# Anony-CFFM/CFFM

Measured on AMD Instinct MI355X. Metric: training examples/sec, frappe 10-field dim32; embedding-gather %HBM roofline, higher is better.
Workload: dtype f32; 1 GPU; frappe shape: synthetic libfm, 10 fields, 5382 features, inner/outer dim 32, batch 256 per GPU, selu, Adagrad lr 0.05, square_loss (README.md:28); global_batch=256, id_distribution=uniform, tables=replicated, parallelism=single

## Files before the change

cffm_amd/csrc/conv.hip:

```cpp
#include <cstdlib>
#include <cstring>

#include "internal.hpp"

#include <type_traits>

#include <stdlib.h>
#include "inner_body.hpp"
#include "head_body.hpp"
#include "sort_body.hpp"

#define KSTEP 32
#define WG_KM 64

__device__ __forceinline__ int64_t xcd_tile(int64_t per_xcd) {
    const int64_t id = blockIdx.x;
    return (id & 7) * per_xcd + (id >> 3);
}
__host__ __device__ static inline int64_t xcd_per(int64_t tiles) { return (tiles + 7) / 8; }

struct RowPos { int b, y, x; };
__device__ __forceinline__ RowPos row_pos(int64_t m, int lgSo) {
    RowPos p;
    const int So = 1 << lgSo;
// ... 1684 lines not shown
                PHASE_MARK(1 + l);
                fused_layer_fwd<NT, G, ACT, LGSO>(fa.conv[l], b, smem, CL(l - 1), CL(l));
            });
        } else {
            for (int l = 1; l < live; ++l) {
                if (lds_act) lds_barrier(); else __syncthreads();
                PHASE_MARK(1 + l);
                fused_layer_fwd<NT, G, ACT>(fa.conv[l], b, smem, CL(l - 1), CL(l));
            }
        }
        if (lds_act) lds_barrier(); else __syncthreads();
        PHASE_MARK(1 + live);
        head_fwd_body<NW, ACT, false, F_, D_>(fa.head, b, smem, lds_act, c0_off, c1_off);
        PHASE_MARK(2 + live);
    };
    if constexpr (CS) {
        static_assert(!CS || 4096 / (CS ? F_ : 1) <= 2 * 256, "two passes over a grid of 256 workgroups cover every accepted B");
        if ((int)blockIdx.x < fa.B) example((int)blockIdx.x);
        if (const int b = blockIdx.x + gridDim.x; b < fa.B) {
            __syncthreads();
            example(b);
        }
    } else {
        for (int b = blockIdx.x; b < fa.B; b += gridDim.x) {
            if (b != (int)blockIdx.x) __syncthreads();
            example(b);
        }
    }
#ifdef CFFM_PHASE_TIMERS
    if (threadIdx.x == 0) cffm_wg_times[2 * blockIdx.x + 1] = wall_clock64();
#endif
}

template <int NT, int F_, int D_, int NW>
__device__ __forceinline__ void conv0_fact_bwd_body(const DgradArgs& a, float* __restrict__ slabW, float* __restrict__ slabB,
                                                    int64_t slab_stride, char* smem, int wg, int nwg) {
    constexpr int PP = NT * 16, S = 16, NTH = 64 * NW, XQ = 16 / NW;
    const int F = F_ ? F_ : a.F, D = D_ ? D_ : a.D, Dp = D + 1, P = F_ ? F_ * (F_ - 1) / 2 : a.P, F2 = 2 * F;
    const int TP = S * PP + 16;
    float* Wl = reinterpret_cast<float*>(smem);
    float* T = Wl + 4 * PP * PP;
    float* part = T + 2 * F * TP;
    float* dEi = part + NW * 16 * 32;
    float* dEj = dEi + 32 * 16;
    float* bred = dEj + 32 * 16;
    float* rs = bred + NW * PP;
    float* Es = rs + 2 * F;
    const int tid = threadIdx.x, lane = tid & 63, wave = tid >> 6, r = lane & 15, kk = lane >> 4;
    float* sw = slabW + (int64_t)wg * slab_stride;
    float* sb = slabB + (int64_t)wg * slab_stride;
    PHASE_MARKB(12, wg);
    {
        const float4* wsrc = reinterpret_cast<const float4*>(a.W);
        for (int i = tid; i < 4 * PP * PP / 4; i += NTH) reinterpret_cast<float4*>(Wl)[i] = wsrc[i];
        for (int e = tid; e < 4 * (PP - P) * PP; e += NTH) {
            const int tap = e / ((PP - P) * PP), o = e - tap * ((PP - P) * PP);
            sw[(tap * PP + P) * PP + o] = 0.f;
        }
    }
    bool first = true;
    float bacc[NT];
#pragma unroll
    for (int nt = 0; nt < NT; ++nt) bacc[nt] = 0.f;

    for (int b = wg; b < a.B; b += nwg) {
        __syncthreads();
        {
// ... 184 lines not shown
                }
            }
#pragma unroll
            for (int ct = 0; ct < 2; ++ct)
#pragma unroll
                for (int j = 0; j < 4; ++j) part[(wave * 16 + kk * 4 + j) * 32 + ct * 16 + r] = acc[ct][j];
        }
        PHASE_MARKB(18, wg);
        if (tid < 2 * F) {
            const int f = tid % F;
            float sacc = 0.f;
            if (tid < F) { for (int h = 0; h < D; ++h) sacc += Es[f * Dp + h]; }
            else { for (int h = 0; h < D; ++h) sacc += Es[f * Dp + h] * a.dt1[(int64_t)b * a.t1w + h]; }
            rs[tid] = sacc;
        }
        __syncthreads();
        for (int e = tid; e < 16 * 32; e += NTH) {
            float v = part[e];
#pragma unroll
            for (int w = 1; w < NW; ++w) v += part[512 * w + e];
            dEj[(e & 31) * 16 + (e >> 5)] = v;
        }
        __syncthreads();
        PHASE_MARKB(19, wg);
        for (int e = tid; e < F * D; e += NTH) {
            const int f = e / D, h = e - f * D, lo = h & 1, hh = h >> 1;
            float R = 0.f, Q = 0.f;
            for (int j = f + 1; j < F; ++j) R += rs[j];
            for (int i = 0; i < f; ++i) Q += rs[F + i];
            a.dprev[(int64_t)b * F * D + e] = (dEi[(lo * F + f) * 16 + hh] + dEj[(lo * F + f) * 16 + hh])
                                              + a.dt1[(int64_t)b * a.t1w + h] * R + Q;
        }
        first = false;
    }
    PHASE_MARKB(20, wg);
    __syncthreads();
#pragma unroll
    for (int nt = 0; nt < NT; ++nt) {
        float v = bacc[nt];
        v += __shfl_xor(v, 16, 64);
        v += __shfl_xor(v, 32, 64);
        if (kk == 0) bred[wave * PP + nt * 16 + r] = v;
    }
    __syncthreads();
    if (tid < PP) {
        float v = bred[tid];
#pragma unroll
        for (int w = 1; w < NW; ++w) v += bred[w * PP + tid];
        sb[tid] = v;
    }
    if (first) {
        for (int e = tid; e < 4 * PP * PP; e += NTH) sw[e] = 0.f;
    }
    PHASE_MARKB(25, wg);
}

template <int NT, int F_, int D_, int NW>
__global__ __launch_bounds__(64 * NW) void conv0_fact_bwd_kernel(DgradArgs a, float* __restrict__ slabW,
                                                              float* __restrict__ slabB, int64_t slab_stride) {
    extern __shared__ __attribute__((aligned(16))) char smem[];
    conv0_fact_bwd_body<NT, F_, D_, NW>(a, slabW, slabB, slab_stride, smem, blockIdx.x, gridDim.x);
}

template <int NT, int RM, bool L0, int HALVES, int ACTC = -1>
__device__ __forceinline__ void dgrad_taps_body(const DgradArgs& a, int wg, char* smem, int64_t m_lo = 0, int64_t m_end = -1,
                                                int tiles = 1, int tid_in = -1) {
// ... 468 lines not shown
struct Conv01Args {
    DgradArgs d0;
    float *slabW0, *slabB0;
    int64_t stride0;
    DgradArgs d1;
    WgradArgs w1, w2, w3;
    int n2, n3;
};

template <int NT, int F_, int D_, int ACT>
__global__ __launch_bounds__(1024) void conv01_bwd_kernel(Conv01Args a) {
    extern __shared__ __attribute__((aligned(16))) char smem[];
    const int b = blockIdx.x, grp = __builtin_amdgcn_readfirstlane((int)(threadIdx.x >> 8)), ltid = threadIdx.x & 255;
    PHASE_MARKB(40, b);
    dgrad_taps_body<NT, 1, false, 4, ACT>(a.d1, b, smem, 0, -1, 4);
    PHASE_MARKB(41, b);
    {
        char* gsm = smem + (size_t)grp * (64 * NT * 16 * 4);
        const WgradArgs& w = grp == 0 ? a.w1 : (grp == 1 ? a.w2 : a.w3);
        const int nsl = grp == 0 ? (int)gridDim.x : (grp == 1 ? a.n2 : a.n3);
        const int slab = grp == 1 ? b - ((int)gridDim.x - a.n2) : b;
        const bool mine = grp < 3 && slab >= 0 && slab < nsl;
        int64_t m_lo = 0, m_hi = 0;
        if (mine) {
            const int64_t per = grp == 0 ? (1ll << (2 * w.lgSo)) : CFFM_TOP_SLAB_ROWS;
            m_lo = (int64_t)slab * per;
            m_hi = min(w.Mtot, m_lo + per);
            if (m_hi < m_lo) m_hi = m_lo;
        }
        wgrad_taps_body<NT, false, 1, ACT>(w, mine ? slab : 0, nsl, gsm, m_lo, m_hi, ltid, mine);
    }
    __syncthreads();
    PHASE_MARKB(42, b);
    conv0_fact_bwd_body<NT, F_, D_, 16>(a.d0, a.slabW0, a.slabB0, a.stride0, smem, b, (int)gridDim.x);
}

struct BwdTopArgs {
    HeadBwdArgs hb;
    DgradArgs d[2];
    WgradArgs w[2];
    int lgSo[2];
    int n_layers;
    int wgrad_here;
    InnerBwdArgs ib;
    int n_inner;
    int n_keys;
    const int32_t* rank_ids;
    unsigned long long* keys_sorted;
    int n_rows;
};

template <int NT, int ACT = -1>
__global__ __launch_bounds__(256) void bwd_top_kernel(BwdTopArgs a) {
    extern __shared__ __attribute__((aligned(16))) char smem[];
    __shared__ float dh1s[CFFM_HEAD_UNITS];
    __shared__ float dt1s[1024];
    __shared__ float red[4];
    const int bid = blockIdx.x;
#ifdef CFFM_PHASE_TIMERS
    if (threadIdx.x == 0) cffm_wg_times[2 * blockIdx.x] = wall_clock64();
#endif
    if (bid < a.n_inner) {
        PHASE_MARKB(36, bid);
        const float L = head_bwd_loss(a.hb, false, red);
        __syncthreads();
        PHASE_MARKB(37, bid);
        if (a.rank_ids != nullptr && a.n_keys == 0) {
            for (int b = bid; b < a.hb.B; b += a.n_inner) rank_keys_body<4>(a.rank_ids, a.n_rows, b, a.hb.g.F, a.hb.g.M, a.keys_sorted, smem);
        }
        PHASE_MARKB(38, bid);
        inner_bwd_body<ACT>(a.ib, bid, a.n_inner, smem, L);
        PHASE_MARKB(39, bid);
#ifdef CFFM_PHASE_TIMERS
        if (threadIdx.x == 0) cffm_wg_times[2 * blockIdx.x + 1] = wall_clock64();
#endif
        return;
    }
    if (bid < a.n_inner + a.n_keys) {
        for (int b = bid - a.n_inner; b < a.hb.B; b += a.n_keys) rank_keys_body<4>(a.rank_ids, a.n_rows, b, a.hb.g.F, a.hb.g.M, a.keys_sorted, smem);
#ifdef CFFM_PHASE_TIMERS
        if (threadIdx.x == 0) cffm_wg_times[2 * blockIdx.x + 1] = wall_clock64();
#endif
        return;
    }
    const int b = bid - a.n_inner - a.n_keys;
    PHASE_MARKB(0, b);
    HeadBwdState st;
    head_bwd_begin(a.hb, b, st);
    PHASE_MARKB(1, b);
    const float L = head_bwd_loss(a.hb, b == 0, red);
    PHASE_MARKB(2, b);
    if (b < a.hb.B)
        head_bwd_example<ACT>(a.hb, b, st, b, head_dout(a.hb.loss, a.hb.out[b], a.hb.y[b], 1.f / (float)a.hb.Bg, L), dh1s, dt1s);
    PHASE_MARKB(3, b);
    head_bwd_end(a.hb, b, st);
    PHASE_MARKB(4, b);
    for (int t = 0; t < a.n_layers; ++t) {
        __syncthreads();
        const int64_t rows = 1ll << (2 * a.lgSo[t]);
        const int64_t m_lo = (int64_t)b * rows, m_hi = b < a.hb.B ? m_lo + rows : m_lo;
        if (a.wgrad_here) wgrad_taps_body<NT, false, 1, ACT>(a.w[t], b, (int)gridDim.x - a.n_inner - a.n_keys, smem, m_lo, m_hi);
        PHASE_MARKB(5 + 2 * t, b);
        for (int64_t m0 = m_lo; m0 < m_hi; m0 += 16) dgrad_taps_body<NT, 1, false, 1, ACT>(a.d[t], 0, smem, m0, m_hi);
        PHASE_MARKB(6 + 2 * t, b);
// ... 1261 lines not shown
        default: return CFFM_ERR_UNSUPPORTED;
    }
}

template <int NT>
static int launch_bwd_top(const BwdTopArgs& a, size_t lds, hipStream_t st) {
    return with_readme_act<NT>(a.hb.g.act, [&](auto act) {
        constexpr int ACT = decltype(act)::value;
        int rc = set_lds(bwd_top_kernel<NT, ACT>, lds);
        if (rc) return rc;
        hipLaunchKernelGGL((bwd_top_kernel<NT, ACT>), dim3(a.n_inner + a.n_keys + 256), dim3(256), lds, st, a);
        CFFM_CHECK_LAUNCH();
        return 0;
    });
}

int cffm_bwd_top_impl(const StepCtx& c, const float* y, int64_t B_global, const BwdOpts& o, hipStream_t st, int* next_layer) {
    const cffm_shape_t* s = c.s;
    const Geo& g = c.g;
    const int32_t B = c.B;
    BwdTopArgs a;
    memset(&a, 0, sizeof(a));
    a.hb = c.head_bwd_args(y, B_global, o);
    const int first = bwd_top_first_layer(s);
    a.wgrad_here = (top_wgrad_deferred(s, B) || bwd_fused01_ok(s, B)) ? 0 : 1;
    a.n_layers = 0;
    for (int l = g.live - 1; l >= first; --l) {
        a.d[a.n_layers] = c.dgrad_args(l);
        a.w[a.n_layers] = c.wgrad_args(l);
        a.lgSo[a.n_layers] = a.d[a.n_layers].lgSo;
        ++a.n_layers;
    }
    a.ib = c.inner_bwd_args(&a.n_inner);
    a.ib.dout = nullptr;
    a.ib.y = y; a.ib.invB = 1.f / (float)B_global;
    if (o.rank_ids != nullptr && s->F <= RANK_MAXF && (int64_t)B * s->F <= 4096) {
        a.rank_ids = o.rank_ids; a.n_rows = B * s->F;
        a.keys_sorted = c.at<unsigned long long>(c.wl.sort_vals);
        a.n_keys = 256;
    }
    size_t lds = (size_t)(WGT_SUB * g.Pp) * 4 + 16;
    if (inner_bwd_lds(g) > lds) lds = inner_bwd_lds(g);
    *next_layer = first - 1;
    return with_int<NT4>(g.Pp / 16, [&](auto nt) { return launch_bwd_top<CV(nt)>(a, lds, st); });
}

int cffm_conv_bwd_impl(const StepCtx& c, int l, hipStream_t st, const ConvBwdOpts& o) {
    const Geo& g = c.g;
    if (l < 0 || l >= g.live) return CFFM_ERR_BAD_SHAPE;
    if (int rc = cffm_conv_lds_check(c)) return rc;
    const SlabRange& sr = c.conv_slab(l);
    const int nsl = sr.nslab;
    WgradArgs wa = c.wgrad_args(l);
    DgradArgs da = c.dgrad_args(l);
    const ConvBwdChoice k = conv_bwd_choice(g, c.B, l, nsl, conv_b3_on());
    const KC &kw = k.wgrad, &kd = k.dgrad;
    if (kw.family == CFFM_CHOICE_UNSUPPORTED || kd.family == CFFM_CHOICE_UNSUPPORTED) return CFFM_ERR_UNSUPPORTED;
    if (o.with_top_wgrad && !k.paired) return CFFM_ERR_UNSUPPORTED;
    const bool tiled_w = kw.family == CFFM_WGRAD_TILE_ALL || kw.family == CFFM_WGRAD_TILE_GROUP;
    if (o.rs && !(tiled_w && kd.family == CFFM_DGRAD_TILE_PACKED)) return CFFM_ERR_UNSUPPORTED;
    if (k.paired) {
        InnerBwdArgs ib{};
        int n_i = 0;
        const bool inner = o.carry_inner != nullptr && c.s->inner_conv;
        if (inner) ib = c.inner_bwd_args(&n_i);
        TopWgrad tw;
// ... 69 lines not shown
extern "C" int cffm_outer_conv0_bwd(const cffm_shape_t* s, const float* theta, void* ws, int32_t B, void* stream) {
    int rc = check_shape(s);
    if (rc) return rc;
    if (B <= 0 || !s->outer_conv) return 0;
    return cffm_conv_bwd_impl(StepCtx(s, B, theta, ws), 0, (hipStream_t)stream);
}
extern "C" int cffm_conv_bwd(const cffm_shape_t* s, const float* theta, void* ws, int32_t B, int32_t layer, void* stream) {
    int rc = check_shape(s);
    if (rc) return rc;
    if (B <= 0 || !s->outer_conv) return 0;
    if (layer < 1) return CFFM_ERR_BAD_SHAPE;
    return cffm_conv_bwd_impl(StepCtx(s, B, theta, ws), layer, (hipStream_t)stream);
}
bool cffm_wide_regather_ok(const cffm_shape_t* s) {
    if (check_shape(s) || !s->inner_conv || !s->outer_conv) return false;
    const Geo g = make_geo(s);
    return conv0_tile_fwd_ok(g) && conv0_tile_wgrad_ok(g) && conv0_tile_dgrad2_ok(g) && g.K == g.D && (g.K == 32 || g.K == 64) &&
           cffm_giw_lds_ok();
}

int cffm_conv01_bwd_impl(const StepCtx& c, hipStream_t st) {
    const cffm_shape_t* s = c.s;
    const Geo& g = c.g;
    const int32_t B = c.B;
    if (!bwd_fused01_ok(s, B) || g.live != 4 || !conv0_fact_bwd_ok(g)) return CFFM_ERR_UNSUPPORTED;
    Conv01Args a;
    memset(&a, 0, sizeof(a));
    const WgradArgs w0 = c.wgrad_args(0);
    a.d0 = c.dgrad_args(0);
    a.slabW0 = w0.slabW; a.slabB0 = w0.slabB; a.stride0 = w0.slab_stride;
    a.d1 = c.dgrad_args(1);
    a.w1 = c.wgrad_args(1); a.w2 = c.wgrad_args(2); a.w3 = c.wgrad_args(3);
    a.n2 = c.conv_slab(2).nslab; a.n3 = c.conv_slab(3).nslab;
    if (c.conv_slab(0).nslab != 256 || c.conv_slab(1).nslab != 256 || a.n2 > 256 || a.n3 > 256 ||
        (int64_t)a.n2 * CFFM_TOP_SLAB_ROWS < a.w2.Mtot || (int64_t)a.n3 * CFFM_TOP_SLAB_ROWS < a.w3.Mtot)
        return CFFM_ERR_UNSUPPORTED;
    {
        const void* must[] = {a.d0.dC, a.d0.W, a.d0.Cprev, a.d0.dt1, a.d0.dprev, a.slabW0, a.slabB0, a.d1.dC, a.d1.W, a.d1.Cprev,
                              a.d1.dt1, a.d1.dprev, a.w1.in, a.w1.dC, a.w1.slabW, a.w1.slabB, a.w2.in, a.w2.dC, a.w2.slabW,
                              a.w2.slabB, a.w3.in, a.w3.dC, a.w3.slabW, a.w3.slabB};
        for (const void* q : must)
            if (q == nullptr) return CFFM_ERR_BAD_SHAPE;
        if (a.d0.Mtot <= 0 || a.d1.Mtot <= 0 || a.w1.Mtot <= 0 || a.w2.Mtot <= 0 || a.w3.Mtot <= 0 || a.n2 < 1 || a.n3 < 1 ||
            a.stride0 <= 0 || a.w1.slab_stride <= 0 || a.w2.slab_stride <= 0 || a.w3.slab_stride <= 0)
            return CFFM_ERR_BAD_SHAPE;
    }
    const int NW = 16, PP = g.Pp;
    const size_t lds = conv0_fact_bwd_lds(PP, g.F, g.D);
#define CFFM_C01_LAUNCH(NTV, FV, DV, ACTV)                                                                       \
    do {                                                                                                         \
        int rc = set_lds(conv01_bwd_kernel<NTV, FV, DV, ACTV>, lds);                                             \
        if (rc) return rc;                                                                                       \
        hipLaunchKernelGGL((conv01_bwd_kernel<NTV, FV, DV, ACTV>), dim3(256), dim3(1024), lds, st, a);          \
    } while (0)
    const int nt = PP / 16;
    if (frappe_shape(g)) CFFM_C01_LAUNCH(3, 10, 32, CFFM_ACT_SELU);
    else if (nt == 3) CFFM_C01_LAUNCH(3, 0, 0, -1);
    else if (nt == 2) CFFM_C01_LAUNCH(2, 0, 0, -1);
    else CFFM_C01_LAUNCH(1, 0, 0, -1);
#undef CFFM_C01_LAUNCH
    CFFM_CHECK_LAUNCH();
    return 0;
}

bool cffm_fwd_all_ok(const cffm_shape_t* s, int32_t B) {
    const Geo g = make_geo(s);
// ... 54 lines not shown
```

cffm_amd/csrc/inner_body.hpp:

```cpp
#pragma once
#include "common.hpp"

struct InnerUnit {
    float x0, x1, I0, I1, z0, z1, s0, s1, eix, eiy, ejx, ejy;
    int i, j;
};

__device__ __forceinline__ InnerUnit inner_unit(const float* E, const uint32_t* lut, int p, int t, int K,
                                                const float* cw, const float* cb, int act) {
    InnerUnit u;
    const uint32_t ij = lut[p];
    u.i = ij & 0xffff; u.j = ij >> 16;
    const float2 ei = *reinterpret_cast<const float2*>(&E[u.i * K + 2 * t]);
    const float2 ej = *reinterpret_cast<const float2*>(&E[u.j * K + 2 * t]);
    u.eix = ei.x; u.eiy = ei.y; u.ejx = ej.x; u.ejy = ej.y;
    u.I0 = ei.x * ej.x; u.I1 = ei.y * ej.y;
    u.x0 = act_f(u.I0, act); u.x1 = act_f(u.I1, act);
    u.z0 = u.x0 * cw[0] + u.x1 * cw[2] + cb[0];
    u.z1 = u.x0 * cw[1] + u.x1 * cw[3] + cb[1];
    const float mp = fmaxf(u.x0, u.x1);
    u.s0 = act_pos(fmaxf(u.z0, 0.f), act) + mp;
    u.s1 = act_pos(fmaxf(u.z1, 0.f), act) + mp;
    return u;
}
// ... 77 lines not shown
    float cw[4] = {cw_g[0], cw_g[1], cw_g[2], cw_g[3]};
    float cb[2] = {cb_g[0], cb_g[1]};
    const int K2 = g.K / 2, units = g.P * K2;
    const float2* wd2 = reinterpret_cast<const float2*>(wd);
    const float2 w2_first = (int)threadIdx.x < units ? wd2[threadIdx.x] : make_float2(0.f, 0.f);
    __syncthreads();
    const float invK2 = 1.f / (float)K2;
    float part = 0.f;
    for (int u = threadIdx.x; u < units; u += blockDim.x) {
        const int p = fast_div(u, invK2), t = u - p * K2;
        const InnerUnit v = inner_unit(E, lut, p, t, g.K, cw, cb, act);
        const float2 w2 = u == (int)threadIdx.x ? w2_first : wd2[u];
        part += v.s0 * w2.x + v.s1 * w2.y;
    }
    const float tot = block_sum(part, red);
    if (threadIdx.x == 0) inner_out[b] = tot + bd[0];
}

struct InnerBwdArgs {
    Geo g;
    int B;
    const float *Ei, *dout, *cw, *cb, *wd;
    const float *out, *y;
    int loss;
    float invB;
    float* dEi;
    float *slab_cw, *slab_cb, *slab_dw, *slab_db;
    int64_t slab_stride;
    const int32_t* idx = nullptr;
    int idxM = 0;
    int idxStride = 0;
};

template <int ACTC = -1>
__device__ __forceinline__ void inner_bwd_body(const InnerBwdArgs& a, int slab, int nslab, char* smem, float L = 1.f) {
    const Geo& g = a.g;
    const int act = ACTC >= 0 ? ACTC : g.act;
    const int B = a.B;
    const float* __restrict__ Ei = a.Ei; const float* __restrict__ dout = a.dout;
    const float* __restrict__ cw_g = a.cw; const float* __restrict__ cb_g = a.cb; const float* __restrict__ wd = a.wd;
    float* __restrict__ dEi = a.dEi;
    float* __restrict__ slab_cw = a.slab_cw + slab * a.slab_stride; float* __restrict__ slab_cb = a.slab_cb + slab * a.slab_stride;
    float* __restrict__ slab_dw = a.slab_dw + slab * a.slab_stride; float* __restrict__ slab_db = a.slab_db + slab * a.slab_stride;
    const int FK = g.F * g.K;
    float* E = reinterpret_cast<float*>(smem);
    float* dE = E + FK;
    uint32_t* lut = reinterpret_cast<uint32_t*>(dE + 4 * FK);
    float* red = reinterpret_cast<float*>(lut + g.Pp);
    const int wave = threadIdx.x >> 6;
    build_pair_lut(lut, g.F, g.Pp);
    if (threadIdx.x < 8) slab_cw[threadIdx.x] = 0.f;
    if (threadIdx.x < 4) slab_db[threadIdx.x] = 0.f;
    float cw[4] = {cw_g[0], cw_g[1], cw_g[2], cw_g[3]};
    float cb[2] = {cb_g[0], cb_g[1]};
    const int K2 = g.K / 2, units = g.P * K2;
    const float invK2 = 1.f / (float)K2;
    float gcw[4] = {0.f, 0.f, 0.f, 0.f}, gcb[2] = {0.f, 0.f}, gdb = 0.f;
    constexpr int UPRE = 4;
    const float2* wd2 = reinterpret_cast<const float2*>(wd);
    float2 w2p[UPRE];
#pragma unroll
    for (int k = 0; k < UPRE; ++k) {
        const int u = threadIdx.x + k * blockDim.x;
        w2p[k] = u < units ? wd2[u] : make_float2(0.f, 0.f);
    }
    bool first = true;
    for (int b = slab; b < B; b += nslab) {
// ... 17 lines not shown
        auto unit_step = [&](int u, float2 w2) {
            const int p = fast_div(u, invK2), t = u - p * K2;
            const InnerUnit v = inner_unit(E, lut, p, t, g.K, cw, cb, act);
            const int64_t wi = (int64_t)p * g.K + 2 * t;
            float2 acc2 = first ? make_float2(0.f, 0.f) : *reinterpret_cast<float2*>(&slab_dw[wi]);
            acc2.x += v.s0 * db; acc2.y += v.s1 * db;
            *reinterpret_cast<float2*>(&slab_dw[wi]) = acc2;
            const float ds0 = db * w2.x, ds1 = db * w2.y;
            const float dz0 = ds0 * act_relu_grad(fmaxf(v.z0, 0.f), act);
            const float dz1 = ds1 * act_relu_grad(fmaxf(v.z1, 0.f), act);
            gcw[0] += dz0 * v.x0; gcw[1] += dz1 * v.x0; gcw[2] += dz0 * v.x1; gcw[3] += dz1 * v.x1;
            gcb[0] += dz0; gcb[1] += dz1;
            const float dmp = ds0 + ds1;
            const bool firstmax = v.x0 >= v.x1;
            const float dx0 = dz0 * cw[0] + dz1 * cw[1] + (firstmax ? dmp : 0.f);
            const float dx1 = dz0 * cw[2] + dz1 * cw[3] + (firstmax ? 0.f : dmp);
            const float dI0 = dx0 * act_grad_f(v.I0, act), dI1 = dx1 * act_grad_f(v.I1, act);
            atomicAdd(&myE[v.i * g.K + 2 * t], dI0 * v.ejx);
            atomicAdd(&myE[v.i * g.K + 2 * t + 1], dI1 * v.ejy);
            atomicAdd(&myE[v.j * g.K + 2 * t], dI0 * v.eix);
            atomicAdd(&myE[v.j * g.K + 2 * t + 1], dI1 * v.eiy);
        };
#pragma unroll
        for (int k = 0; k < UPRE; ++k) {
            const int u = threadIdx.x + k * blockDim.x;
            if (u < units) unit_step(u, w2p[k]);
        }
        for (int u = threadIdx.x + UPRE * blockDim.x; u < units; u += blockDim.x) unit_step(u, wd2[u]);
        if (threadIdx.x == 0) gdb += db;
        __syncthreads();
        for (int i = threadIdx.x; i < FK; i += blockDim.x)
            dEi[(int64_t)b * FK + i] = ((dE[i] + dE[FK + i]) + dE[2 * FK + i]) + dE[3 * FK + i];
        first = false;
    }
    if (first) {
        for (int64_t i = threadIdx.x; i < (int64_t)g.P * g.K; i += blockDim.x) slab_dw[i] = 0.f;
    }
    float r[7] = {gcw[0], gcw[1], gcw[2], gcw[3], gcb[0], gcb[1], gdb};
#pragma unroll
    for (int q = 0; q < 7; ++q) r[q] = wave_sum(r[q]);
    __syncthreads();
    if ((threadIdx.x & 63) == 0) {
#pragma unroll
        for (int q = 0; q < 7; ++q) dE[wave * 8 + q] = r[q];
    }
    __syncthreads();
    if (threadIdx.x == 0) {
        const int nw = blockDim.x >> 6;
#pragma unroll
        for (int q = 0; q < 7; ++q) {
            float t = 0.f;
            for (int w = 0; w < nw; ++w) t += dE[w * 8 + q];
            r[q] = t;
        }
        for (int q = 0; q < 4; ++q) slab_cw[q] = r[q];
        slab_cb[0] = r[4]; slab_cb[1] = r[5];
        slab_db[0] = r[6];
    }
}
```

cffm_amd/csrc/optim.hip:

```cpp
#include "internal.hpp"

#include <cmath>
#include <cstring>
#include <rocprim/device/device_radix_sort.hpp>

#define REDUCE_GROUPS 64
static inline int reduce_slab_wgs(int64_t n) { return (int)((n / 4 + REDUCE_GROUPS - 1) / REDUCE_GROUPS); }
__device__ __forceinline__ void reduce_slabs_body(int bid, const float* __restrict__ gpart, int64_t n, const SlabPlan& sp,
                                                  float* __restrict__ grad, float* __restrict__ theta,
                                                  float* __restrict__ acc, float lr) {
    __shared__ float4 part[4][REDUCE_GROUPS];
    const int g = threadIdx.x & 63, q = threadIdx.x >> 6;
    const int64_t i = ((int64_t)bid * REDUCE_GROUPS + g) * 4;
    float4 s = make_float4(0.f, 0.f, 0.f, 0.f);
    if (i < n) {
        int hit = 0;
        for (int r = 1; r < sp.n; ++r)
            if (i >= sp.r[r].off) hit = r;
        const SlabRange rg = sp.r[hit];
        const float4* src = reinterpret_cast<const float4*>(gpart + rg.base + (i - rg.off));
        const int64_t stride = rg.len / 4;
        const int per = (rg.nslab + 3) / 4, k0 = q * per, k1 = min(rg.nslab, k0 + per);
#pragma unroll 8
        for (int k = k0; k < k1; ++k) {
            const float4 v = src[(int64_t)k * stride];
            s.x += v.x; s.y += v.y; s.z += v.z; s.w += v.w;
        }
    }
    part[q][g] = s;
    __syncthreads();
    if (q != 0 || i >= n) return;
#pragma unroll
    for (int e = 1; e < 4; ++e) {
        const float4 p = part[e][g];
        s.x += p.x; s.y += p.y; s.z += p.z; s.w += p.w;
    }
    *reinterpret_cast<float4*>(grad + i) = s;
    if (theta != nullptr) {
        float4 a = *reinterpret_cast<float4*>(acc + i), t = *reinterpret_cast<float4*>(theta + i);
        a.x += s.x * s.x; a.y += s.y * s.y; a.z += s.z * s.z; a.w += s.w * s.w;
        t.x -= lr * s.x / sqrtf(a.x); t.y -= lr * s.y / sqrtf(a.y); t.z -= lr * s.z / sqrtf(a.z); t.w -= lr * s.w / sqrtf(a.w);
        *reinterpret_cast<float4*>(acc + i) = a;
        *reinterpret_cast<float4*>(theta + i) = t;
    }
}

__global__ __launch_bounds__(256) void reduce_slabs_kernel(const float* __restrict__ gpart, int64_t n, SlabPlan sp,
                                                           float* __restrict__ grad, float* __restrict__ theta,
                                                           float* __restrict__ acc, float lr) {
    reduce_slabs_body(blockIdx.x, gpart, n, sp, grad, theta, acc, lr);
}

__device__ __forceinline__ float late_scale(const LateScale& ls) {
    return ls.on ? 1.f / sqrtf(ls.sum[0] * ls.inv_Bg + 1e-10f) : 1.f;
}

struct AdagradRule {
    float lr;
    __device__ __forceinline__ bool slot() const { return true; }
// ... 203 lines not shown
    return 0;
}

__global__ __launch_bounds__(256) void pack_keys_kernel(const int32_t* __restrict__ ids, unsigned long long* keys, int64_t n,
                                                        int64_t id_stride, int M) {
    const int64_t i = (int64_t)blockIdx.x * 256 + threadIdx.x;
    if (i < n) {
        const int raw = ids[i * id_stride];
        keys[i] = ((unsigned long long)(unsigned)((raw < 0 || raw >= M) ? M : raw) << 32) | (unsigned long long)i;
    }
}

#include "sort_body.hpp"

__global__ __launch_bounds__(256) void small_sort_kernel(const unsigned long long* __restrict__ in,
                                                         unsigned long long* __restrict__ out, int n, int id_bits) {
    extern __shared__ __attribute__((aligned(16))) char smem[];
    small_sort_body(in, nullptr, out, n, id_bits, smem);
}

struct SparseArgs {
    const unsigned long long* keys;
    int64_t n;
    int M, K, D;
    const float *dEi, *dEo, *dfb;
    int64_t sEi, sEo, sfb;
    int run_len;
    int64_t run_stride;
    float inv_run_len;
};
enum { T_INNER = 0, T_OUTER = 1, T_BIAS = 2 };
static const cffm_tables_t NO_TABLES = {nullptr, nullptr, nullptr};

template <class Sink>
__device__ __forceinline__ void segment_walk(int bid, const SparseArgs& a, const Sink& sink) {
    const unsigned long long* __restrict__ keys = a.keys;
    const int64_t n = a.n;
    const int M = a.M, K = a.K, D = a.D;
    const float* __restrict__ dEi = a.dEi; const float* __restrict__ dEo = a.dEo; const float* __restrict__ dfb = a.dfb;
    const int64_t pos = (int64_t)bid * 4 + (threadIdx.x >> 6);
    const int lane = threadIdx.x & 63;
    if (pos >= n) return;
    const int id = (int)(keys[pos] >> 32);
    if (pos > 0 && (int)(keys[pos - 1] >> 32) == id) return;
    if (id < 0 || id >= M) return;
    const int W = (dEi ? K : 0) + (dEo ? D : 0) + 1;
    const int Ki = dEi ? K : 0;
    for (int c0 = 0; c0 < W; c0 += 64) {
        const int c = c0 + lane;
        float g = 0.f;
        if (c < W) {
            for (int64_t q = pos; q < n; ++q) {
                const unsigned long long kq = keys[q];
                if ((int)(kq >> 32) != id) break;
                int64_t sl = (int64_t)(kq & 0xffffffffull);
                int64_t boff = 0;
                if (a.run_len > 0) {
                    const int blk = fast_div((int)sl, a.inv_run_len);
                    boff = (int64_t)blk * a.run_stride;
                    sl -= (int64_t)blk * a.run_len;
                }
                g += c < Ki ? dEi[boff + sl * a.sEi + c] : (c < W - 1 ? dEo[boff + sl * a.sEo + (c - Ki)] : dfb[boff + sl * a.sfb]);
            }
            typename Sink::At at;
            if (c < Ki) at = sink.at(id, T_INNER, c);
            else if (c < W - 1) at = sink.at(id, T_OUTER, c - Ki);
            else at = sink.at(id, T_BIAS, 0);
            sink(at, g);
        }
    }
}

__device__ __forceinline__ int64_t row_off(int K, int D, int id, int t, int col) {
    if (t == T_INNER) return (int64_t)id * K + col;
    if (t == T_OUTER) return (int64_t)id * D + col;
    return id;
}
__device__ __forceinline__ float* table_of(const cffm_tables_t& T, int t) {
    if (t == T_INNER) return T.inner_emb;
    if (t == T_OUTER) return T.outer_emb;
    return T.feat_bias;
}
template <class Rule, bool LATE>
struct ApplySink {
    cffm_tables_t w, s;
    int K, D;
    Rule rule;
    float gscale = 1.f;
    struct At { float *w, *s; };
    __device__ __forceinline__ At at(int id, int t, int col) const {
        const int64_t o = row_off(K, D, id, t, col);
        return {table_of(w, t) + o, rule.slot() ? table_of(s, t) + o : nullptr};
    }
    __device__ __forceinline__ void operator()(const At& a, float g) const {
        if (LATE) g *= gscale;
        rule(*a.w, a.s, nullptr, g);
    }
};
struct StoreSink {
    cffm_tables_t G;
    int K, D;
    typedef float* At;
    __device__ __forceinline__ At at(int id, int t, int col) const { return table_of(G, t) + row_off(K, D, id, t, col); }
    __device__ __forceinline__ void operator()(At a, float g) const { *a = g; }
};
template <class Rule>
struct MixSink {
    ApplySink<Rule, false> apply;
    StoreSink store;
    int store_mask;
    struct At { typename ApplySink<Rule, false>::At a; float* G; };
    __device__ __forceinline__ At at(int id, int t, int col) const {
        if ((store_mask >> t) & 1) return {{nullptr, nullptr}, store.at(id, t, col)};
        return {apply.at(id, t, col), nullptr};
    }
    __device__ __forceinline__ void operator()(const At& a, float g) const {
        if (a.G) store(a.G, g);
        else apply(a.a, g);
    }
};

struct ApplyArgs { cffm_tables_t w, s; LateScale ls; };
template <class Rule>
__device__ __forceinline__ void sparse_apply_body(int bid, const SparseArgs& a, const ApplyArgs& p, const Rule& rule) {
    segment_walk(bid, a, ApplySink<Rule, true>{p.w, p.s, a.K, a.D, rule, late_scale(p.ls)});
}
template <class Rule>
__global__ __launch_bounds__(256) void sparse_apply_kernel(SparseArgs a, ApplyArgs p, Rule rule) { sparse_apply_body(blockIdx.x, a, p, rule); }

__global__ __launch_bounds__(256) void update_all_kernel(const float* __restrict__ gpart, int64_t n, SlabPlan sp,
                                                         float* __restrict__ grad, float* __restrict__ theta,
                                                         float* __restrict__ acc, float lr, int n_reduce, SparseArgs sa, ApplyArgs pa) {
    if ((int)blockIdx.x < n_reduce) {
        PHASE_MARKB(26, blockIdx.x);
        reduce_slabs_body(blockIdx.x, gpart, n, sp, grad, theta, acc, lr);
        PHASE_MARKB(27, blockIdx.x);
    } else {
        PHASE_MARKB(28, blockIdx.x - n_reduce);
        sparse_apply_body(blockIdx.x - n_reduce, sa, pa, AdagradRule{lr});
        PHASE_MARKB(29, blockIdx.x - n_reduce);
    }
}
#ifdef CFFM_PHASE_TIMERS
extern "C" int cffm_debug_upd_times(unsigned long long* host32) {
    return (int)hipMemcpyFromSymbol(host32, HIP_SYMBOL(cffm_bwd_times), sizeof(cffm_bwd_times));
}
#endif

extern "C" int cffm_reduce_slabs(const cffm_shape_t* s, void* ws, int32_t B, float* grad, void* stream) {
    int rc = check_shape(s);
    if (rc) return rc;
// ... 308 lines not shown
```

Measured before the change: 2.916 million examples/s.

## Restructure sparse segment walk, pipeline slab reduction loads, single-pass backward bodies

Rewrites the sparse segment walk so a wave reads 64 sorted keys per ballot, broadcasts slot indices with readlane, batches gradient gathers in groups of up to eight, and prefetches the table row and optimizer state before the sum. The slab reduction drops its data-dependent range search for a predicated unrolled select and keeps a ring of sixteen float4 loads in flight, using asm pins to stop the compiler from reordering the adds. The inner and conv0 backward bodies break after one example, and the host rejects B above 256 so that assumption holds. The aim is more memory-level parallelism in the gather and reduce phases, paid for with higher register pressure and new launch restrictions.

Result: faster. 2.984 million examples/s, median of 6 (+2.3%).

```diff
diff --git a/cffm_amd/csrc/conv.hip b/cffm_amd/csrc/conv.hip
--- a/cffm_amd/csrc/conv.hip
+++ b/cffm_amd/csrc/conv.hip
@@ -1740,7 +1740,7 @@
 #endif
 }
 
-template <int NT, int F_, int D_, int NW>
+template <int NT, int F_, int D_, int NW, bool ONE = false>
 __device__ __forceinline__ void conv0_fact_bwd_body(const DgradArgs& a, float* __restrict__ slabW, float* __restrict__ slabB,
                                                     int64_t slab_stride, char* smem, int wg, int nwg) {
     constexpr int PP = NT * 16, S = 16, NTH = 64 * NW, XQ = 16 / NW;
@@ -1991,6 +1991,7 @@
                                               + a.dt1[(int64_t)b * a.t1w + h] * R + Q;
         }
         first = false;
+        if constexpr (ONE) break;
     }
     PHASE_MARKB(20, wg);
     __syncthreads();
@@ -2525,7 +2526,7 @@
     }
     __syncthreads();
     PHASE_MARKB(42, b);
-    conv0_fact_bwd_body<NT, F_, D_, 16>(a.d0, a.slabW0, a.slabB0, a.stride0, smem, b, (int)gridDim.x);
+    conv0_fact_bwd_body<NT, F_, D_, 16, true>(a.d0, a.slabW0, a.slabB0, a.stride0, smem, b, (int)gridDim.x);
 }
 
 struct BwdTopArgs {
@@ -2562,7 +2563,7 @@
             for (int b = bid; b < a.hb.B; b += a.n_inner) rank_keys_body<4>(a.rank_ids, a.n_rows, b, a.hb.g.F, a.hb.g.M, a.keys_sorted, smem);
         }
         PHASE_MARKB(38, bid);
-        inner_bwd_body<ACT>(a.ib, bid, a.n_inner, smem, L);
+        inner_bwd_body<ACT, true>(a.ib, bid, a.n_inner, smem, L);
         PHASE_MARKB(39, bid);
 #ifdef CFFM_PHASE_TIMERS
         if (threadIdx.x == 0) cffm_wg_times[2 * blockIdx.x + 1] = wall_clock64();
@@ -3890,6 +3891,7 @@
         ++a.n_layers;
     }
     a.ib = c.inner_bwd_args(&a.n_inner);
+    if (B > a.n_inner || B > 256) return CFFM_ERR_UNSUPPORTED;
     a.ib.dout = nullptr;
     a.ib.y = y; a.ib.invB = 1.f / (float)B_global;
     if (o.rank_ids != nullptr && s->F <= RANK_MAXF && (int64_t)B * s->F <= 4096) {
@@ -4025,6 +4027,7 @@
     a.d1 = c.dgrad_args(1);
     a.w1 = c.wgrad_args(1); a.w2 = c.wgrad_args(2); a.w3 = c.wgrad_args(3);
     a.n2 = c.conv_slab(2).nslab; a.n3 = c.conv_slab(3).nslab;
+    if (B > 256) return CFFM_ERR_UNSUPPORTED;
     if (c.conv_slab(0).nslab != 256 || c.conv_slab(1).nslab != 256 || a.n2 > 256 || a.n3 > 256 ||
         (int64_t)a.n2 * CFFM_TOP_SLAB_ROWS < a.w2.Mtot || (int64_t)a.n3 * CFFM_TOP_SLAB_ROWS < a.w3.Mtot)
         return CFFM_ERR_UNSUPPORTED;
diff --git a/cffm_amd/csrc/inner_body.hpp b/cffm_amd/csrc/inner_body.hpp
--- a/cffm_amd/csrc/inner_body.hpp
+++ b/cffm_amd/csrc/inner_body.hpp
@@ -133,7 +133,7 @@
     int idxStride = 0;
 };
 
-template <int ACTC = -1>
+template <int ACTC = -1, bool ONE = false>
 __device__ __forceinline__ void inner_bwd_body(const InnerBwdArgs& a, int slab, int nslab, char* smem, float L = 1.f) {
     const Geo& g = a.g;
     const int act = ACTC >= 0 ? ACTC : g.act;
@@ -217,6 +217,7 @@
         for (int i = threadIdx.x; i < FK; i += blockDim.x)
             dEi[(int64_t)b * FK + i] = ((dE[i] + dE[FK + i]) + dE[2 * FK + i]) + dE[3 * FK + i];
         first = false;
+        if constexpr (ONE) break;
     }
     if (first) {
         for (int64_t i = threadIdx.x; i < (int64_t)g.P * g.K; i += blockDim.x) slab_dw[i] = 0.f;
diff --git a/cffm_amd/csrc/optim.hip b/cffm_amd/csrc/optim.hip
--- a/cffm_amd/csrc/optim.hip
+++ b/cffm_amd/csrc/optim.hip
@@ -2,9 +2,12 @@
 
 #include <cmath>
 #include <cstring>
+#include <type_traits>
 #include <rocprim/device/device_radix_sort.hpp>
 
 #define REDUCE_GROUPS 64
+#define REDUCE_RING 16
+#define REDUCE_PIN(s) asm volatile("" : "+v"((s).x), "+v"((s).y), "+v"((s).z), "+v"((s).w) : : "memory")
 static inline int reduce_slab_wgs(int64_t n) { return (int)((n / 4 + REDUCE_GROUPS - 1) / REDUCE_GROUPS); }
 __device__ __forceinline__ void reduce_slabs_body(int bid, const float* __restrict__ gpart, int64_t n, const SlabPlan& sp,
                                                   float* __restrict__ grad, float* __restrict__ theta,
@@ -14,17 +17,47 @@
     const int64_t i = ((int64_t)bid * REDUCE_GROUPS + g) * 4;
     float4 s = make_float4(0.f, 0.f, 0.f, 0.f);
     if (i < n) {
-        int hit = 0;
-        for (int r = 1; r < sp.n; ++r)
-            if (i >= sp.r[r].off) hit = r;
-        const SlabRange rg = sp.r[hit];
-        const float4* src = reinterpret_cast<const float4*>(gpart + rg.base + (i - rg.off));
-        const int64_t stride = rg.len / 4;
-        const int per = (rg.nslab + 3) / 4, k0 = q * per, k1 = min(rg.nslab, k0 + per);
-#pragma unroll 8
-        for (int k = k0; k < k1; ++k) {
-            const float4 v = src[(int64_t)k * stride];
-            s.x += v.x; s.y += v.y; s.z += v.z; s.w += v.w;
+        int64_t rel = sp.r[0].base - sp.r[0].off, len = sp.r[0].len;
+        int nslab = sp.r[0].nslab;
+#pragma unroll
+        for (int r = 1; r < CFFM_MAX_LAYERS + 3; ++r) {
+            const bool hit = r < sp.n && i >= sp.r[r].off;
+            rel = hit ? sp.r[r].base - sp.r[r].off : rel; len = hit ? sp.r[r].len : len; nslab = hit ? sp.r[r].nslab : nslab;
+        }
+        const int64_t stride = len / 4;
+        const int per = (nslab + 3) / 4, k0 = q * per, k1 = min(nslab, k0 + per);
+        if (k0 < k1) {
+            const float4* p = reinterpret_cast<const float4*>(gpart + rel + i) + (int64_t)k0 * stride;
+            float4 v[REDUCE_RING];
+#pragma unroll
+            for (int j = 0; j < REDUCE_RING; ++j) {
+                v[j] = *p;
+                p += k0 + j + 1 < k1 ? stride : 0;
+            }
+            int k = k0;
+            for (; k + 2 * REDUCE_RING <= k1; k += REDUCE_RING) {
+#pragma unroll
+                for (int j = 0; j < REDUCE_RING; ++j) {
+                    s.x += v[j].x; s.y += v[j].y; s.z += v[j].z; s.w += v[j].w;
+                    REDUCE_PIN(s);
+                    v[j] = *p;
+                    p += stride;
+                }
+            }
+            if (k + REDUCE_RING < k1) {
+#pragma unroll
+                for (int j = 0; j < REDUCE_RING; ++j) {
+                    s.x += v[j].x; s.y += v[j].y; s.z += v[j].z; s.w += v[j].w;
+                    REDUCE_PIN(s);
+                    v[j] = *p;
+                    p += k + REDUCE_RING + j + 1 < k1 ? stride : 0;
+                }
+                k += REDUCE_RING;
+            }
+#pragma unroll
+            for (int j = 0; j < REDUCE_RING; ++j) {
+                if (k + j < k1) { s.x += v[j].x; s.y += v[j].y; s.z += v[j].z; s.w += v[j].w; }
+            }
         }
     }
     part[q][g] = s;
@@ -294,43 +327,84 @@
 enum { T_INNER = 0, T_OUTER = 1, T_BIAS = 2 };
 static const cffm_tables_t NO_TABLES = {nullptr, nullptr, nullptr};
 
+template <int NCH, class Sink>
+__device__ __forceinline__ void segment_walk_cols(const SparseArgs& a, const Sink& sink, int64_t pos, unsigned long long kq, int id,
+                                                  int c0, int W, int Ki, int lane) {
+    const unsigned long long* __restrict__ keys = a.keys;
+    const int64_t n = a.n;
+    const float* gp[NCH];
+    int64_t gs[NCH];
+    typename Sink::At at[NCH];
+    typename Sink::Pre pre[NCH];
+    float g[NCH];
+    bool live[NCH];
+#pragma unroll
+    for (int ch = 0; ch < NCH; ++ch) {
+        const int c = c0 + ch * 64 + lane;
+        live[ch] = c < W;
+        const int cc = live[ch] ? c : W - 1;
+        const bool in_i = cc < Ki, in_o = !in_i && cc < W - 1;
+        const typename Sink::At ai = sink.at(id, T_INNER, in_i ? cc : 0), ao = sink.at(id, T_OUTER, in_o ? cc - Ki : 0),
+                                ab = sink.at(id, T_BIAS, 0);
+        gp[ch] = in_i ? a.dEi + cc : (in_o ? a.dEo + (cc - Ki) : a.dfb);
+        gs[ch] = in_i ? a.sEi : (in_o ? a.sEo : a.sfb);
+        at[ch] = in_i ? ai : (in_o ? ao : ab);
+        pre[ch] = sink.pre(at[ch]);
+        g[ch] = 0.f;
+    }
+    for (int64_t q0 = pos;; q0 += 64) {
+        if (q0 != pos) kq = q0 + lane < n ? keys[q0 + lane] : ~0ull;
+        const unsigned long long in_run = __ballot((int)(kq >> 32) == id);
+        const int cnt = ~in_run == 0ull ? 64 : __builtin_ctzll(~in_run);
+        int sl = (int)(unsigned)(kq & 0xffffffffull), blk = 0;
+        if (a.run_len > 0) {
+            blk = fast_div(sl, a.inv_run_len);
+            sl -= blk * a.run_len;
+        }
+        auto slots = [&](int j, auto N) {
+            float v[decltype(N)::value][NCH];
+#pragma unroll
+            for (int t = 0; t < decltype(N)::value; ++t) {
+                const int64_t s = __builtin_amdgcn_readlane(sl, j + t);
+                const int64_t boff = (int64_t)__builtin_amdgcn_readlane(blk, j + t) * a.run_stride;
+#pragma unroll
+                for (int ch = 0; ch < NCH; ++ch) v[t][ch] = gp[ch][boff + s * gs[ch]];
+            }
+#pragma unroll
+            for (int t = 0; t < decltype(N)::value; ++t)
+#pragma unroll
+                for (int ch = 0; ch < NCH; ++ch) g[ch] += v[t][ch];
+        };
+        int j = 0;
+        for (; j + 8 <= cnt; j += 8) slots(j, std::integral_constant<int, 8>());
+        if (cnt & 4) { slots(j, std::integral_constant<int, 4>()); j += 4; }
+        if (cnt & 2) { slots(j, std::integral_constant<int, 2>()); j += 2; }
+        if (cnt & 1) slots(j, std::integral_constant<int, 1>());
+        if (cnt < 64) break;
+    }
+#pragma unroll
+    for (int ch = 0; ch < NCH; ++ch)
+        if (live[ch]) sink(at[ch], pre[ch], g[ch]);
+}
+
 template <class Sink>
 __device__ __forceinline__ void segment_walk(int bid, const SparseArgs& a, const Sink& sink) {
     const unsigned long long* __restrict__ keys = a.keys;
     const int64_t n = a.n;
-    const int M = a.M, K = a.K, D = a.D;
-    const float* __restrict__ dEi = a.dEi; const float* __restrict__ dEo = a.dEo; const float* __restrict__ dfb = a.dfb;
     const int64_t pos = (int64_t)bid * 4 + (threadIdx.x >> 6);
     const int lane = threadIdx.x & 63;
     if (pos >= n) return;
-    const int id = (int)(keys[pos] >> 32);
-    if (pos > 0 && (int)(keys[pos - 1] >> 32) == id) return;
-    if (id < 0 || id >= M) return;
-    const int W = (dEi ? K : 0) + (dEo ? D : 0) + 1;
-    const int Ki = dEi ? K : 0;
-    for (int c0 = 0; c0 < W; c0 += 64) {
-        const int c = c0 + lane;
-        float g = 0.f;
-        if (c < W) {
-            for (int64_t q = pos; q < n; ++q) {
-                const unsigned long long kq = keys[q];
-                if ((int)(kq >> 32) != id) break;
-                int64_t sl = (int64_t)(kq & 0xffffffffull);
-                int64_t boff = 0;
-                if (a.run_len > 0) {
-                    const int blk = fast_div((int)sl, a.inv_run_len);
-                    boff = (int64_t)blk * a.run_stride;
-                    sl -= (int64_t)blk * a.run_len;
-                }
-                g += c < Ki ? dEi[boff + sl * a.sEi + c] : (c < W - 1 ? dEo[boff + sl * a.sEo + (c - Ki)] : dfb[boff + sl * a.sfb]);
-            }
-            typename Sink::At at;
-            if (c < Ki) at = sink.at(id, T_INNER, c);
-            else if (c < W - 1) at = sink.at(id, T_OUTER, c - Ki);
-            else at = sink.at(id, T_BIAS, 0);
-            sink(at, g);
-        }
-    }
+    const unsigned long long kq = pos + lane < n ? keys[pos + lane] : ~0ull;
+    const int id_prev = (int)(keys[pos > 0 ? pos - 1 : 0] >> 32);
+    const int id = __builtin_amdgcn_readfirstlane((int)(kq >> 32));
+    if (pos > 0 && id_prev == id) return;
+    if (id < 0 || id >= a.M) return;
+    const int W = (a.dEi ? a.K : 0) + (a.dEo ? a.D : 0) + 1;
+    const int Ki = a.dEi ? a.K : 0;
+    if (W <= 64) segment_walk_cols<1>(a, sink, pos, kq, id, 0, W, Ki, lane);
+    else if (W <= 128) segment_walk_cols<2>(a, sink, pos, kq, id, 0, W, Ki, lane);
+    else
+        for (int c0 = 0; c0 < W; c0 += 256) segment_walk_cols<4>(a, sink, pos, kq, id, c0, W, Ki, lane);
 }
 
 __device__ __forceinline__ int64_t row_off(int K, int D, int id, int t, int col) {
@@ -350,21 +424,28 @@
     Rule rule;
     float gscale = 1.f;
     struct At { float *w, *s; };
+    struct Pre { float w, s; };
     __device__ __forceinline__ At at(int id, int t, int col) const {
         const int64_t o = row_off(K, D, id, t, col);
         return {table_of(w, t) + o, rule.slot() ? table_of(s, t) + o : nullptr};
     }
-    __device__ __forceinline__ void operator()(const At& a, float g) const {
+    __device__ __forceinline__ Pre pre(const At& a) const { return {*a.w, rule.slot() ? *a.s : 0.f}; }
+    __device__ __forceinline__ void operator()(const At& a, const Pre& p, float g) const {
         if (LATE) g *= gscale;
-        rule(*a.w, a.s, nullptr, g);
+        float wv = p.w, sv = p.s;
+        rule(wv, &sv, nullptr, g);
+        if (rule.slot()) *a.s = sv;
+        *a.w = wv;
     }
 };
 struct StoreSink {
     cffm_tables_t G;
     int K, D;
     typedef float* At;
+    struct Pre {};
     __device__ __forceinline__ At at(int id, int t, int col) const { return table_of(G, t) + row_off(K, D, id, t, col); }
-    __device__ __forceinline__ void operator()(At a, float g) const { *a = g; }
+    __device__ __forceinline__ Pre pre(At) const { return {}; }
+    __device__ __forceinline__ void operator()(At a, const Pre&, float g) const { *a = g; }
 };
 template <class Rule>
 struct MixSink {
@@ -376,9 +457,11 @@
         if ((store_mask >> t) & 1) return {{nullptr, nullptr}, store.at(id, t, col)};
         return {apply.at(id, t, col), nullptr};
     }
-    __device__ __forceinline__ void operator()(const At& a, float g) const {
-        if (a.G) store(a.G, g);
-        else apply(a.a, g);
+    typedef typename ApplySink<Rule, false>::Pre Pre;
+    __device__ __forceinline__ Pre pre(const At& a) const { return a.G ? Pre{0.f, 0.f} : apply.pre(a.a); }
+    __device__ __forceinline__ void operator()(const At& a, const Pre& p, float g) const {
+        if (a.G) store(a.G, StoreSink::Pre(), g);
+        else apply(a.a, p, g);
     }
 };
 
```
